# openjamoses/TOSEM-2021-Replication

Measured on NVIDIA H100. Metric: source MB/s scanned (tokenise + line-hash + classify + aggregate), higher is better.
Workload: dtype u8

## Files before the change

### tosem-2021-replication_b200/csrc/tsm_api.cu

```cuda
#include <algorithm>
#include <cstdio>
#include <cstdlib>
#include <cstring>
#include <chrono>
#include <new>
#include <utility>
#include <vector>

#include "tsm_device.cuh"

#include "tsm_scan_kernels.cuh"
#include "tsm_scan_walk.cuh"
#include "tsm_reduce_kernels.cuh"
#include "tsm_diff_kernels.cuh"
#include "tsm_blame_kernels.cuh"
#include "tsm_stmt_kernels.cuh"
#include "tsm_lines_kernels.cuh"
#include "tsm_similar_kernels.cuh"
#include "tsm_clone_kernels.cuh"
#include "tsm_case_kernels.cuh"
#include "tsm_edit_kernels.cuh"

using namespace tsm;

// ... 351 lines not shown
  rc = upload_index(c, k, st);
  if (rc != TSM_OK) return rc;
  if (c->n_files) CU(cudaMemcpyAsync(c->d_arena, k->arena, (size_t)c->arena_bytes, cudaMemcpyHostToDevice, st));
  c->resident = true;
  c->scanned = false;
  return TSM_OK;
}

static int ensure_event_buffers(tsm_ctx* c, uint32_t flags) {
  if ((flags & TSM_SCAN_ASSERT_EVENTS) && !c->d_aev)
    CU(cudaMalloc((void**)&c->d_aev, sizeof(tsm_assert_event) * (size_t)c->max_events));
  if ((flags & TSM_SCAN_HEADER_EVENTS) && !c->d_hev)
    CU(cudaMalloc((void**)&c->d_hev, sizeof(tsm_header_event) * (size_t)c->max_events));
  return TSM_OK;
}

static ScanParams make_params(const tsm_ctx* c, uint32_t flags) {
  ScanParams p{};
  p.arena = c->d_arena; p.off = c->d_off; p.len = c->d_len; p.ext = c->d_ext; p.grp = c->d_grp;
  p.n_files = c->n_files; p.n_groups = c->n_groups;
  p.unit_file = c->d_unit_file; p.unit_begin = c->d_unit_begin; p.unit_cap = c->unit_cap;
  p.ctrl = c->d_ctrl; p.stats = c->d_stats;
  p.cand = c->d_cand; p.cand_cap = (uint32_t)c->max_events;
  p.hev = c->d_hev; p.hev_cap = (uint32_t)c->max_events;
  p.aev = c->d_aev; p.aev_cap = (uint32_t)c->max_events;
  p.counts = c->d_counts; p.flags = flags; p.four = 4; p.cls_last = 1;
  return p;
}

static void launch_k_scan(const tsm_ctx* c, const ScanParams& p, bool rev_b, cudaStream_t st) {
  if (rev_b) k_scan_t<true><<<c->sms * SCAN2_CTAS_PER_SM, SCAN2_WARPS * 32, SCAN2_SMEM_B, st>>>(p);
  else k_scan_t<false><<<c->sms * SCAN2_CTAS_PER_SM, SCAN2_WARPS * 32, SCAN2_SMEM, st>>>(p);
}

struct ClassifyShape { size_t smem; uint32_t wave; };
static ClassifyShape classify_shape(tsm_ctx* c, int32_t n_groups) {
  const size_t smem = CLS_SMEM_BASE + sizeof(uint32_t) * (n_groups <= 16 ? (size_t)n_groups * TSM_K : 0);
  if (c->cls_smem != smem) {
    int per_sm = 0;
    if (cudaOccupancyMaxActiveBlocksPerMultiprocessor(&per_sm, k_classify_t<false>, 256, smem) != cudaSuccess || per_sm < 1) per_sm = 4;
    c->cls_per_sm = per_sm;
    c->cls_smem = smem;
  }
  return {smem, (uint32_t)(c->sms * c->cls_per_sm)};
}

static void launch_k_classify(const ScanParams& p, bool rev_b, uint32_t grid, size_t smem, cudaStream_t st) {
  if (rev_b) k_classify_t<true><<<grid, 256, smem, st>>>(p);
  else k_classify_t<false><<<grid, 256, smem, st>>>(p);
}

static int launch_scan(tsm_ctx* c, uint32_t flags, cudaStream_t st, const tsm_corpus* host, bool check_files_here = false) {
  int rc = ensure_event_buffers(c, flags);
  if (rc != TSM_OK) return rc;
  ScanParams p = make_params(c, flags);
  const int n = c->n_files;
  c->launches = 0;
  CU(cudaMemsetAsync(c->d_zero, 0, (size_t)(reinterpret_cast<uint8_t*>(c->d_counts) - c->d_zero) +
                     sizeof(unsigned long long) * ((size_t)(c->n_groups + 1) * TSM_K + 4), st));
  if (n) {
    std::vector<int32_t> cut{0};
    if (host) {
      int64_t slab_bytes = 32ll << 20;
      while (c->arena_bytes / slab_bytes + 1 > tsm_ctx::kMaxSlabs) slab_bytes *= 2;
      int64_t next = slab_bytes;
      for (int32_t i = 1; i < n; ++i)
        if ((int64_t)host->off[i] >= next) { cut.push_back(i); next = (int64_t)host->off[i] + slab_bytes; }
      CU(cudaEventRecord(c->ready_ev, st));
      CU(cudaStreamWaitEvent(c->copy_stream, c->ready_ev, 0));
    }
    cut.push_back(n);
    if ((int)cut.size() - 1 > tsm_ctx::kMaxSlabs) return TSM_E_LAYOUT;
    const int es = c->ev_next;
    c->ev_next = (es + 1) % tsm_ctx::kRing;
    fold_events(c, es);
    cudaEvent_t* ev = c->ev[es];
    CU(cudaEventRecord(ev[0], st));
    const int n_slabs = (int)cut.size() - 1;
    const bool rev_b = flags & TSM_SCAN_REV_B;
    const ClassifyShape cls = classify_shape(c, c->n_groups);
    for (int s = 0; s < n_slabs; ++s) {
      const int32_t f0 = cut[(size_t)s], f1 = cut[(size_t)s + 1];
      if (host) {
        if (check_files_here && s == 0) {
          const int rc0 = check_files(host, f0, f1, true, true);
          if (rc0 != TSM_OK) return rc0;
        }
        const size_t b0 = (size_t)host->off[f0], b1 = (size_t)host->off[f1];
        CU(cudaMemcpyAsync(c->d_arena + b0, host->arena + b0, b1 - b0, cudaMemcpyHostToDevice, c->copy_stream));
        CU(cudaEventRecord(c->slab_ev[s], c->copy_stream));
        CU(cudaStreamWaitEvent(st, c->slab_ev[s], 0));
        if (check_files_here && s + 1 < n_slabs) {
          const int rc1 = check_files(host, f1, cut[(size_t)s + 2], true, true);
          if (rc1 != TSM_OK) { cudaStreamSynchronize(c->copy_stream); cudaStreamSynchronize(st); return rc1; }
        }
      }
      p.slab = c->d_slab + s; p.f_begin = f0; p.f_end = f1;
      p.unit_base = (uint32_t)((host ? (int64_t)host->off[f0] : 0) / CH + f0);
      k_plan<<<(f1 - f0 + 255) / 256, 256, 0, st>>>(p);
      CU(cudaGetLastError());
      if (s == 0 && n_slabs == 1) CU(cudaEventRecord(ev[1], st));
      launch_k_scan(c, p, rev_b, st);
      CU(cudaGetLastError());
      if (s + 1 < n_slabs) {
        p.cls_last = 0;
        launch_k_classify(p, rev_b, cls.wave, cls.smem, st);
        CU(cudaGetLastError());
        p.cls_last = 1;
      }
    }
    if (n_slabs > 1) CU(cudaEventRecord(ev[1], st));
    CU(cudaEventRecord(ev[2], st));
    launch_k_classify(p, rev_b, cls.wave, cls.smem, st);
    CU(cudaGetLastError());
    CU(cudaEventRecord(ev[3], st));
    CU(cudaEventRecord(ev[4], st));
    c->ev_used[es] = (n_slabs == 1);
    c->ev_last = es;
    c->launches = 3 * n_slabs;
    CU(cudaGetLastError());
  }
  c->last_flags = flags;
  c->scanned = true;
  return TSM_OK;
}

extern "C" int tsm_scan_resident(tsm_ctx* c, uint32_t flags, void* stream) {
  if (!c) return TSM_E_ARG;
  flags &= TSM_SCAN_ASSERT_EVENTS | TSM_SCAN_HEADER_EVENTS | TSM_SCAN_REV_B;
  if (!c->resident) return TSM_E_STATE;
  CallScope call(c, (cudaStream_t)stream);
  CU(call.status);
  return launch_scan(c, flags, (cudaStream_t)stream, nullptr);
}

extern "C" int tsm_device_counts(tsm_ctx* c, void** dptr, int64_t* n_int64) {
  if (!c || !dptr || !n_int64) return TSM_E_ARG;
  if (!c->scanned) return TSM_E_STATE;
  *dptr = c->d_counts;
  *n_int64 = (int64_t)(c->n_groups + 1) * TSM_K + 4;
  return TSM_OK;
}

extern "C" int tsm_last_launch_count(tsm_ctx* c) { return c ? c->launches : 0; }

#if TSM_PHASE_CLOCKS
extern "C" int tsm_phase_clocks(unsigned long long* out, int n, int reset) {
  if (!out || n < (int)PH_N) return TSM_E_ARG;
  CU(cudaDeviceSynchronize());
  CU(cudaMemcpyFromSymbol(out, g_scan_phase_clk, sizeof(unsigned long long) * PH_N));
  if (reset) {
    const unsigned long long zero[PH_N] = {};
    CU(cudaMemcpyToSymbol(g_scan_phase_clk, zero, sizeof(zero)));
  }
  return TSM_OK;
}
#endif

extern "C" int tsm_last_kernel_ms(tsm_ctx* c, float* ms4) {
  if (!c || !ms4) return TSM_E_ARG;
  if (!c->scanned || c->n_files == 0 || c->ev_last < 0) return TSM_E_STATE;
  CU(cudaSetDevice(c->device));
  cudaEvent_t* ev = c->ev[c->ev_last];
  CU(cudaEventSynchronize(ev[4]));
  for (int i = 0; i < 4; ++i) CU(cudaEventElapsedTime(&ms4[i], ev[i], ev[i + 1]));
  return TSM_OK;
}

extern "C" int tsm_kernel_ms_stats(tsm_ctx* c, double* sum_ms4, int64_t* n_scans, int reset) {
  if (!c) return TSM_E_ARG;
  CU(cudaSetDevice(c->device));
  for (int i = 0; i < tsm_ctx::kRing; ++i) fold_events(c, i);
  if (sum_ms4) for (int k = 0; k < 4; ++k) sum_ms4[k] = c->ms_sum[k];
  if (n_scans) *n_scans = c->ms_n;
  if (reset) { for (double& v : c->ms_sum) v = 0; c->ms_n = 0; }
  return TSM_OK;
}

static int grow_event_buffers(tsm_ctx* c, int64_t need) {
  if (need <= c->max_events) return TSM_OK;
  if (need > 0xFFFFFFF0ll) return TSM_E_CAPACITY;
  unsigned long long* cand = nullptr;
  tsm_assert_event* aev = nullptr;
  tsm_header_event* hev = nullptr;
  const bool ok = cudaMalloc((void**)&cand, sizeof(unsigned long long) * (size_t)need) == cudaSuccess &&
                  (!c->d_aev || cudaMalloc((void**)&aev, sizeof(tsm_assert_event) * (size_t)need) == cudaSuccess) &&
                  (!c->d_hev || cudaMalloc((void**)&hev, sizeof(tsm_header_event) * (size_t)need) == cudaSuccess);
  if (!ok) {
    cudaGetLastError();
    cudaFree(cand); cudaFree(aev); cudaFree(hev);
    return TSM_E_CUDA;
  }
  cudaFree(c->d_cand); cudaFree(c->d_aev); cudaFree(c->d_hev);
  c->d_cand = cand; c->d_aev = aev; c->d_hev = hev;
  c->max_events = need;
  return TSM_OK;
}

static int download_tables(tsm_ctx* c, tsm_result* r, cudaStream_t st) {
  const int n = c->n_files, G = c->n_groups;
  unsigned long long* h_tot = reinterpret_cast<unsigned long long*>(c->h_ctrl + 1);
  CU(cudaMemcpyAsync(c->h_ctrl, c->d_ctrl, sizeof(Ctrl), cudaMemcpyDeviceToHost, st));
  CU(cudaMemcpyAsync(h_tot, c->d_counts + (size_t)(G + 1) * TSM_K, 4 * sizeof(unsigned long long), cudaMemcpyDeviceToHost, st));
  if (r->stats && n) CU(cudaMemcpyAsync(r->stats, c->d_stats, sizeof(tsm_file_stat) * (size_t)n, cudaMemcpyDeviceToHost, st));
  if (r->group_counts) CU(cudaMemcpyAsync(r->group_counts, c->d_counts, sizeof(int64_t) * (size_t)G * TSM_K, cudaMemcpyDeviceToHost, st));
  if (r->global_counts) CU(cudaMemcpyAsync(r->global_counts, c->d_counts + (size_t)G * TSM_K, sizeof(int64_t) * TSM_K, cudaMemcpyDeviceToHost, st));
  CU(cudaStreamSynchronize(st));
  for (int i = 0; i < 4; ++i) r->totals[i] = (int64_t)h_tot[i];
  return TSM_OK;
}

template <typename Event> static void sort_events_by_file(Event* ev, uint32_t m, int32_t n_files) {
  if (m < 2) return;
  std::vector<uint32_t> pos((size_t)n_files + 1, 0);
  for (uint32_t i = 0; i < m; ++i) pos[(size_t)ev[i].file + 1]++;
  for (int32_t f = 0; f < n_files; ++f) pos[(size_t)f + 1] += pos[(size_t)f];
  std::vector<Event> tmp(m);
  std::vector<uint32_t> at(pos.begin(), pos.end() - 1);
  for (uint32_t i = 0; i < m; ++i) tmp[at[ev[i].file]++] = ev[i];
  for (int32_t f = 0; f < n_files; ++f)
    if (pos[(size_t)f + 1] - pos[(size_t)f] > 1)
      std::sort(tmp.begin() + pos[(size_t)f], tmp.begin() + pos[(size_t)f + 1],
                [](const Event& a, const Event& b) { return a.line_off < b.line_off; });
  std::copy(tmp.begin(), tmp.end(), ev);
}

static int download(tsm_ctx* c, tsm_result* r, cudaStream_t st) {
  r->n_aev = 0; r->n_hev = 0;
  int rc = download_tables(c, r, st);
  if (rc != TSM_OK) return rc;
  if (c->h_ctrl->overflow) {
    const Ctrl& k = *c->h_ctrl;
    rc = grow_event_buffers(c, std::max<int64_t>(k.n_cand, std::max(k.n_hev, k.n_aev)));
    if (rc == TSM_OK) rc = launch_scan(c, c->last_flags, st, nullptr);
    if (rc == TSM_OK) rc = download_tables(c, r, st);
    if (rc != TSM_OK) return rc;
    if (c->h_ctrl->overflow) return TSM_E_CAPACITY;
  }
  const bool want_aev = (c->last_flags & TSM_SCAN_ASSERT_EVENTS) && r->aev, want_hev = (c->last_flags & TSM_SCAN_HEADER_EVENTS) && r->hev;
  if ((want_aev && (int64_t)c->h_ctrl->n_aev > r->aev_cap) || (want_hev && (int64_t)c->h_ctrl->n_hev > r->hev_cap)) {
    r->n_aev = c->h_ctrl->n_aev; r->n_hev = c->h_ctrl->n_hev;
    return TSM_E_CAPACITY;
  }
  if (want_aev) {
    const uint32_t m = c->h_ctrl->n_aev;
    CU(cudaMemcpyAsync(r->aev, c->d_aev, sizeof(tsm_assert_event) * (size_t)m, cudaMemcpyDeviceToHost, st));
    CU(cudaStreamSynchronize(st));
    sort_events_by_file(r->aev, m, c->n_files);
    r->n_aev = m;
  } else if (c->last_flags & TSM_SCAN_ASSERT_EVENTS) r->n_aev = c->h_ctrl->n_aev;
  if (want_hev) {
    const uint32_t m = c->h_ctrl->n_hev;
    CU(cudaMemcpyAsync(r->hev, c->d_hev, sizeof(tsm_header_event) * (size_t)m, cudaMemcpyDeviceToHost, st));
    CU(cudaStreamSynchronize(st));
    sort_events_by_file(r->hev, m, c->n_files);
    r->n_hev = m;
  } else if (c->last_flags & TSM_SCAN_HEADER_EVENTS) r->n_hev = c->h_ctrl->n_hev;
  return TSM_OK;
}

extern "C" int tsm_download(tsm_ctx* c, tsm_result* r, void* stream) {
  if (!c || !r) return TSM_E_ARG;
  if (!c->scanned) return TSM_E_STATE;
  CallScope call(c, (cudaStream_t)stream);
  CU(call.status);
  return download(c, r, (cudaStream_t)stream);
}

extern "C" int tsm_scan(tsm_ctx* c, const tsm_corpus* k, tsm_result* r, uint32_t flags, void* stream) {
  if (!c || !r) return TSM_E_ARG;
  int rc = check_corpus_head(c, k);
  if (rc != TSM_OK) return rc;
  flags &= TSM_SCAN_ASSERT_EVENTS | TSM_SCAN_HEADER_EVENTS | TSM_SCAN_REV_B;
  cudaStream_t st = (cudaStream_t)stream;
  CallScope call(c, st);
  CU(call.status);
  rc = upload_index(c, k, st);
  if (rc != TSM_OK) return rc;
  c->resident = true;
  rc = launch_scan(c, flags, st, k, true);
  if (rc != TSM_OK) { c->resident = false; c->scanned = false; return rc; }
  return download(c, r, st);
}

extern "C" int tsm_reduce(tsm_ctx* c, const uint8_t* flags, const int32_t* repo, const int32_t* case_id,
                          int32_t n_rows, int32_t n_flags, int32_t n_repos, int32_t n_cases,
                          int64_t* out, int64_t* cases_per_repo, void* stream) {
  if (!c || n_rows < 0 || n_flags < 0 || n_repos <= 0 || n_cases <= 0 || !out || (n_rows && (!flags || !repo || !case_id)))
    return TSM_E_ARG;
  for (int32_t i = 0; i < n_rows; ++i)
    if (repo[i] < 0 || repo[i] >= n_repos || case_id[i] < 0 || case_id[i] >= n_cases) return TSM_E_ARG;
  cudaStream_t st = (cudaStream_t)stream;
  CallScope call(c, st);
  CU(call.status);
  const size_t words = ((size_t)n_cases + 31) / 32;
  const size_t nbits = (size_t)(n_flags + 1) * n_repos * words;
  DevBuf b_flags, b_repo, b_case, b_bits, b_out;
  SyncGuard guard(st);
  if (!b_flags.alloc((size_t)n_rows * n_flags) || !b_repo.alloc(sizeof(int32_t) * (size_t)n_rows) ||
      !b_case.alloc(sizeof(int32_t) * (size_t)n_rows) || !b_bits.alloc(sizeof(uint32_t) * nbits) ||
      !b_out.alloc(sizeof(unsigned long long) * (size_t)(n_flags + 1) * n_repos))
    return TSM_E_CUDA;
  uint8_t* d_flags = b_flags.as<uint8_t>(); int32_t *d_repo = b_repo.as<int32_t>(), *d_case = b_case.as<int32_t>();
  uint32_t* d_bits = b_bits.as<uint32_t>();
  unsigned long long* d_out = b_out.as<unsigned long long>();
  int rc = TSM_OK;
// ... 1193 lines not shown
```

### tosem-2021-replication_b200/csrc/tsm_scan_kernels.cuh

```cuda
#pragma once
#include "tsm_device.cuh"

namespace tsm {

__constant__ uint32_t c_lut[256];
__constant__ uint32_t c_lut_b[256];
__constant__ uint32_t c_elut[256];
__device__ uint8_t c_cat_slot[TSM_CAT_SLOTS];
__device__ uint16_t c_cat_off[TSM_CAT_NAMED + 1];
__device__ char c_cat_blob[TSM_CAT_BLOB_LEN + 1];

__global__ void k_plan(ScanParams p) {
  const int f = p.f_begin + blockIdx.x * blockDim.x + threadIdx.x;
  const int lane = threadIdx.x & 31;
  if (blockIdx.x == 0 && threadIdx.x == 0) p.ctrl->cls_done = p.ctrl->n_cand;
  uint32_t nu = 0;
  if (f < p.f_end) {
    nu = ((uint32_t)p.len[f] + CH - 1) / CH;
    if (nu != 1) p.stats[f] = tsm_file_stat{0, 0, 0, 0, 0};
  }
  uint32_t incl = nu;
#pragma unroll
  for (int d = 1; d < 32; d <<= 1) {
    uint32_t t = __shfl_up_sync(0xffffffffu, incl, d);
    if (lane >= d) incl += t;
  }
  const uint32_t total = __shfl_sync(0xffffffffu, incl, 31);
  uint32_t base = 0;
  if (lane == 31 && total) base = atomicAdd(&p.slab->n_units, total);
  base = __shfl_sync(0xffffffffu, base, 31);
  uint32_t at = p.unit_base + base + incl - nu;
  for (uint32_t u = 0; u < nu; ++u, ++at) {
    if (at < p.unit_cap) { p.unit_file[at] = (uint32_t)f; p.unit_begin[at] = u * CH; }
    else p.ctrl->overflow = 1;
  }
}

__device__ __forceinline__ uint32_t nl_word(uint32_t w) {
  const uint32_t y = w ^ 0x0A0A0A0Au;
  const uint32_t t = (y & 0x7F7F7F7Fu) + 0x7F7F7F7Fu;
  const uint32_t z = ~(t | y | 0x7F7F7F7Fu);
  return (z * 0x00204081u) >> 28;
}
__device__ __forceinline__ uint32_t spaces_of(unsigned long long w) {
  const unsigned long long x = w ^ 0x2020202020202020ull, k7 = 0x7F7F7F7F7F7F7F7Full;
  const unsigned long long nz = (((x & k7) + k7) | x) & ~k7;
  return nz ? ((uint32_t)__ffsll((long long)nz) - 1u) >> 3 : 8u;
}
struct SmemByte {
  const uint8_t* b;
  __device__ __forceinline__ uint32_t operator()(uint32_t i) const { return b[i]; }
  __device__ __forceinline__ unsigned long long load8(uint32_t i) const {
    const uint32_t a = i & ~7u, sh = 8u * (i & 7u);
    const unsigned long long lo = *reinterpret_cast<const unsigned long long*>(b + a);
    const unsigned long long hi = *reinterpret_cast<const unsigned long long*>(b + a + 8);
    return sh ? (lo >> sh) | (hi << (64u - sh)) : lo;
  }
  __device__ __forceinline__ uint32_t spaces8(uint32_t i) const { return spaces_of(load8(i)); }
};
struct HbmByte {
  const uint8_t* b;
  __device__ __forceinline__ uint32_t operator()(uint32_t i) const { return __ldg(b + i); }
  __device__ __forceinline__ unsigned long long load8(uint32_t i) const {
    const unsigned long long* w = reinterpret_cast<const unsigned long long*>(b) + (i >> 3);
    const uint32_t sh = 8u * (i & 7u);
    const unsigned long long lo = __ldg(w), hi = __ldg(w + 1);
    return sh ? (lo >> sh) | (hi << (64u - sh)) : lo;
  }
  __device__ __forceinline__ uint32_t spaces8(uint32_t i) const { return spaces_of(load8(i)); }
};
struct Accum { uint32_t lines, asserts, hdrs, fixes; unsigned long long digest; };

__device__ __forceinline__ uint32_t warp_reserve(uint32_t* counter, uint32_t n, int lane) {
  uint32_t base = 0;
  if (lane == 0 && n) base = atomicAdd(counter, n);
  return __shfl_sync(0xffffffffu, base, 0);
}

__device__ __forceinline__ const uint32_t* scan_lut() {
  extern __shared__ __align__(128) uint8_t smem[];
  return reinterpret_cast<const uint32_t*>(smem);
}

__device__ __forceinline__ void issue_load(const ScanParams& p, uint8_t* buf, uint64_t* bar, uint32_t fo,
                                           uint32_t size, uint32_t cb) {
  const uint32_t lb = cb ? cb - PRE : 0u;
  const uint32_t le = min(cb + CH + EXT, size);
  const uint32_t bytes = (le - lb + 15u) & ~15u;
  mbar_expect_tx(bar, bytes);
  bulk_load(buf + PRE - (cb - lb), p.arena + (size_t)fo + lb, bytes, bar);
}

struct Unit { uint32_t u, f, cb, fo, size; int ext; };

__device__ __forceinline__ Unit claim_unit(const ScanParams& p, uint32_t n_units, int lane) {
  Unit x{0, 0, 0, 0, 0, 0};
  if (lane == 0) x.u = atomicAdd(&p.slab->work, 1u);
  x.u = __shfl_sync(0xffffffffu, x.u, 0);
  if (x.u < n_units) {
    x.f = p.unit_file[p.unit_base + x.u];
    x.cb = p.unit_begin[p.unit_base + x.u];
    x.fo = (uint32_t)p.off[x.f];
    x.size = (uint32_t)p.len[x.f];
    x.ext = p.ext[x.f];
  }
  return x;
}

constexpr uint32_t CC_W = 1, CC_IDENT = 2, CC_STOP = 4;
constexpr uint32_t CLS_CAT_OFF_N = (TSM_CAT_NAMED + 2) & ~1u;
constexpr uint32_t CLS_CAT_WORDS = ((TSM_CAT_SLOTS + 2 * CLS_CAT_OFF_N + TSM_CAT_BLOB_LEN + 15) / 16) * 4;
constexpr uint32_t CLS_SMEM_BASE = 4 * (512 + CLS_CAT_WORDS + 4 * 1024 + 4);
constexpr uint32_t E_FIRST = (1u << 0) | (1u << 5) | (1u << 9) | (1u << 17) | (1u << 21) | (1u << 23) | (1u << 25) |
                             (1u << 27) | (1u << 29) | (1u << 30);

struct FileBytes {
  const unsigned long long* base; uint32_t cur_blk; unsigned long long w;
  uint32_t blk0; unsigned long long w0, w1, w2, w3;
  __device__ __forceinline__ FileBytes(const uint8_t* b, uint32_t first_byte)
      : base(reinterpret_cast<const unsigned long long*>(b)), cur_blk(0xFFFFFFFFu), w(0), blk0(first_byte >> 3) {
    w0 = __ldg(base + blk0); w1 = __ldg(base + blk0 + 1); w2 = __ldg(base + blk0 + 2); w3 = __ldg(base + blk0 + 3);
  }
  __device__ __forceinline__ unsigned long long word(uint32_t blk) const {
    const uint32_t d = blk - blk0;
    if (d < 4u) return d < 2u ? (d == 0u ? w0 : w1) : (d == 2u ? w2 : w3);
    return __ldg(base + blk);
  }
  __device__ __forceinline__ uint32_t get(uint32_t i) {
    const uint32_t blk = i >> 3;
    if (blk != cur_blk) { w = word(blk); cur_blk = blk; }
    return (uint32_t)(w >> (8u * (i & 7u))) & 0xFFu;
  }
  __device__ __forceinline__ unsigned long long get8(uint32_t i) const {
    const uint32_t blk = i >> 3, sh = 8u * (i & 7u);
    const unsigned long long lo = word(blk);
    if (sh == 0) return lo;
    return (lo >> sh) | (word(blk + 1) << (64u - sh));
  }
};

__device__ __forceinline__ unsigned long long low_bytes(unsigned long long v, uint32_t n) {
  return n >= 8 ? v : (v & ((1ull << (8u * n)) - 1ull));
}

__device__ __forceinline__ int stem_lookup(FileBytes& rd, uint32_t s, uint32_t n) {
  if (n < 2 || n > 9) return 0;
  const unsigned long long v = low_bytes(rd.get8(s), n);
  const uint32_t c9 = n == 9 ? rd.get(s + 8) : 0u;
  switch (n) {
    case 2:
      if (v == 0x5145ull) return 1;
      if (v == 0x454Eull) return 2;
      if (v == 0x5447ull) return 5;
      if (v == 0x4547ull) return 6;
      if (v == 0x544Cull) return 7;
      if (v == 0x454Cull) return 8;
      return 0;
    case 4:
      if (v == 0x45555254ull) return 3;
      if (v == 0x5241454Eull) return 9;
      return 0;
    case 5:
      if (v == 0x45534C4146ull) return 4;
      if (v == 0x574F524854ull) return 12;
      return 0;
    case 8: return v == 0x51455F54414F4C46ull ? 10 : 0;
    case 9: return (v == 0x455F454C42554F44ull && c9 == 'Q') ? 11 : 0;
    default: return 0;
  }
}

__device__ __forceinline__ int bare_assert_category(FileBytes& rd, uint32_t e0, uint32_t en, const uint32_t* elut, int deflt = 3,
                                                    bool not_prefix = true) {
  if (not_prefix && en >= 4 && (uint32_t)rd.get8(e0) == 0x20746F6Eu) return 2;
  uint32_t D = 0, A = 0;
  for (uint32_t a = 0; a < en; a += 8) {
    unsigned long long w = rd.get8(e0 + a);
    if (en - a < 8) w &= (1ull << (8u * (en - a))) - 1ull;
    const uint32_t lo = (uint32_t)w, hi = (uint32_t)(w >> 32);
#pragma unroll
    for (int k = 0; k < 4; ++k) { D = ((D + D) | E_FIRST) & elut[__byte_perm(lo, 0, 0x4440 + k)]; A |= D; }
#pragma unroll
    for (int k = 0; k < 4; ++k) { D = ((D + D) | E_FIRST) & elut[__byte_perm(hi, 0, 0x4440 + k)]; A |= D; }
  }
  if (((A & (1u << 4)) && (A & (1u << 8))) || (A & (1u << 16))) return 4;
  if (A & (1u << 20)) return 3;
  if (A & (1u << 22)) return 1;
  if (A & (1u << 24)) return 2;
  if (A & (1u << 26)) return 8;
  if (A & (1u << 28)) return 6;
  if (A & (1u << 29)) return 7;
  if (A & (1u << 30)) return 5;
  return deflt;
}

__device__ __noinline__ bool ident_eq(FileBytes& rd, uint32_t s, uint32_t n, const char* name, uint32_t len) {
  if (n != len) return false;
  for (uint32_t k = 0; k < len; ++k)
    if (rd.get(s + k) != (uint8_t)name[k]) return false;
  return true;
}

constexpr uint32_t BQ_CAP = 1024;

#ifndef TSM_CLS_MINB
#define TSM_CLS_MINB 1
#endif
template <bool REVB>
__global__ void __launch_bounds__(256, TSM_CLS_MINB) k_classify_t(ScanParams p) {
  extern __shared__ __align__(16) uint32_t csm[];
  uint32_t* cls = csm;
  uint32_t* elut = csm + 256;
  uint8_t* cat_slot = reinterpret_cast<uint8_t*>(csm + 512);
  uint16_t* cat_off = reinterpret_cast<uint16_t*>(cat_slot + TSM_CAT_SLOTS);
  uint8_t* cat_blob = reinterpret_cast<uint8_t*>(cat_off + CLS_CAT_OFF_N);
  uint4* bq = reinterpret_cast<uint4*>(csm + 512 + CLS_CAT_WORDS);
  uint32_t* bqn = csm + 512 + CLS_CAT_WORDS + 4 * BQ_CAP;
  uint32_t* hist = bqn + 4;
  const bool use_smem = p.n_groups <= 16;
  for (int i = threadIdx.x; i < 256; i += blockDim.x) {
    const uint32_t c = (uint32_t)i;
    cls[i] = (is_w(c) ? CC_W : 0u) | (is_ident(c) ? CC_IDENT : 0u) | ((c == '(' || c == '\n') ? CC_STOP : 0u);
    elut[i] = c_elut[i];
  }
  for (int i = threadIdx.x; i < TSM_CAT_SLOTS; i += blockDim.x) cat_slot[i] = c_cat_slot[i];
  for (int i = threadIdx.x; i < TSM_CAT_NAMED + 1; i += blockDim.x) cat_off[i] = c_cat_off[i];
  for (int i = threadIdx.x; i < TSM_CAT_BLOB_LEN; i += blockDim.x) cat_blob[i] = (uint8_t)c_cat_blob[i];
  if (use_smem) for (int i = threadIdx.x; i < p.n_groups * TSM_K; i += blockDim.x) hist[i] = 0;
  if (threadIdx.x == 0) *bqn = 0;
  __syncthreads();
  auto count = [&](uint32_t f, int cat) {
    const uint32_t g = p.grp ? p.grp[f] : 0u;
    if (use_smem) atomicAdd(&hist[g * TSM_K + cat], 1u);
    else {
      atomicAdd(&p.counts[(size_t)g * TSM_K + cat], 1ull);
      atomicAdd(&p.counts[(size_t)p.n_groups * TSM_K + cat], 1ull);
    }
  };
  const uint32_t n = min(p.ctrl->n_cand, p.cand_cap), n0 = min(p.ctrl->cls_done, n);
  const bool want_ev = (p.flags & TSM_SCAN_ASSERT_EVENTS) != 0;
  constexpr bool revb = REVB;
  for (uint32_t i = n0 + blockIdx.x * blockDim.x + threadIdx.x; i < n; i += gridDim.x * blockDim.x) {
    const unsigned long long cd = p.cand[i];
    const uint32_t f = (uint32_t)(cd >> 32), line_off = (uint32_t)cd;
    const uint32_t size = (uint32_t)p.len[f];
    FileBytes rd(p.arena + (size_t)(uint32_t)p.off[f], line_off);
    uint32_t q = line_off;
    while (q < size && (cls[rd.get(q)] & CC_W)) ++q;
    const uint32_t t0 = q;
    uint32_t stop = size;
    for (uint32_t wb = t0 & ~7u; wb < size; wb += 8) {
      unsigned long long w = rd.word(wb >> 3);
      const unsigned long long x1 = w ^ 0x2828282828282828ull, x2 = w ^ 0x0A0A0A0A0A0A0A0Aull;
      const unsigned long long k7 = 0x7F7F7F7F7F7F7F7Full;
      unsigned long long z = (~(((x1 & k7) + k7) | x1 | k7)) | (~(((x2 & k7) + k7) | x2 | k7));
      if (wb < t0) z &= ~0ull << (8u * (t0 - wb));
      if (z) { stop = wb + ((uint32_t)__ffsll((long long)z) - 1u) / 8u; break; }
    }
    stop = min(stop, size);
    uint32_t last = stop;
    while (last > t0 && (cls[rd.get(last - 1)] & CC_W)) --last;
    uint32_t Ls = last;
    while (Ls > t0 && (cls[rd.get(Ls - 1)] & CC_IDENT)) --Ls;
    uint32_t tlen = last - t0;
    const uint32_t tlen_a = tlen, Ln = last - Ls;
    int cat = 0;
    bool done = false;
    uint32_t def_e0 = 0, def_en = 0;
    if (revb) {
      const bool macro = ident_eq(rd, Ls, Ln, "BOOST_CHECK", 11) || ident_eq(rd, Ls, Ln, "NTA_CHECK", 9);
      const bool bare6 = tlen == 6 && low_bytes(rd.get8(t0), 6) == 0x747265737361ull;
      const bool full = macro || p.ext[f] == TSM_EXT_JAVA;
      uint32_t fe = last;
      if (full || ((macro || bare6) && stop < size && rd.get(stop) == '(')) {
        uint32_t le = stop;
        while (le < size && rd.get(le) != '\n') ++le;
        fe = le;
        while (fe > t0 && (cls[rd.get(fe - 1)] & CC_W)) --fe;
      }
      if (ident_eq(rd, Ls, Ln, "BOOST_CHECK_EQUAL", 17)) { cat = 1; done = true; }
      else if ((macro || bare6) && stop < size && rd.get(stop) == '(') {
        uint32_t x = stop + 1;
        while (x < fe && (cls[rd.get(x)] & CC_W)) ++x;
        if (x < fe && rd.get(x) == '!' && !(x + 1 < fe && rd.get(x + 1) == '=')) cat = 4;
        else cat = bare_assert_category(rd, x, fe > x ? fe - x : 0u, elut, macro ? 0 : 3, false);
        done = true;
      }
      if (full) tlen = fe - t0;
    }
    if (Ln >= 7) {
      const unsigned long long h7 = low_bytes(rd.get8(Ls), 7);
      if (h7 == 0x5F544345505845ull || h7 == 0x5F545245535341ull) { cat = stem_lookup(rd, Ls + 7, Ln - 7); done = true; }
    }
    if (!done && tlen_a >= 6) {
      const unsigned long long h = rd.get8(t0);
      const bool a6 = low_bytes(h, 6) == 0x747265737361ull;
      if (a6 && tlen_a == 6) { cat = 3; done = true; }
      else if (a6 && tlen_a >= 8 && ((h >> 48) & 0xFF) == 0x20) {
        done = true;
        def_e0 = t0 + 7; def_en = tlen_a - 7;
      }
    }
    if (!done && Ln >= 6) {
      const unsigned long long h = rd.get8(Ls);
      if (low_bytes(h, 6) == 0x747265737361ull) {
        if (Ln == 7 && ((h >> 48) & 0xFF) == '_') cat = 3;
        else {
          cat = TSM_CAT_OTHER;
          uint32_t hh = 0x811C9DC5u;
          for (uint32_t j = 0; j < Ln; j += 8) {
            unsigned long long w = rd.get8(Ls + j);
            const uint32_t nb = min(8u, Ln - j);
#pragma unroll
            for (uint32_t k = 0; k < 8; ++k) {
              if (k < nb) hh = (hh ^ ((uint32_t)w & 0xFFu)) * 0x01000193u;
              w >>= 8;
            }
          }
          const int id = cat_slot[(hh * TSM_CAT_HASH_MULT) >> 23];
          if (id && (uint32_t)(cat_off[id + 1] - cat_off[id]) == Ln) {
            const uint8_t* name = cat_blob + cat_off[id];
            bool ok = true;
            for (uint32_t j = 0; j < Ln; j += 8) {
              unsigned long long w = rd.get8(Ls + j);
              const uint32_t nb = min(8u, Ln - j);
              for (uint32_t k = 0; k < nb; ++k) { ok &= ((uint32_t)w & 0xFFu) == (uint32_t)name[j + k]; w >>= 8; }
            }
            if (ok) cat = id;
          }
        }
      }
    }
    uint32_t ev_slot = 0xFFFFFFFFu;
    if (want_ev) {
      unsigned long long hacc = 0; uint32_t hr = 0;
      for (uint32_t j = 0; j < tlen; ++j) {
        hacc = fold61(hacc + rotl61((unsigned long long)rd.get(t0 + j), hr));
        hr += 8; if (hr >= 61) hr -= 61;
      }
      const uint32_t slot = atomicAdd(&p.ctrl->n_aev, 1u);
      if (slot < p.aev_cap) {
        tsm_assert_event ev;
        ev.file = f; ev.line_off = line_off; ev.stmt_off = t0;
        ev.stmt_len = (uint16_t)min(tlen, 65535u); ev.cat = (uint16_t)cat;
        ev.ident_off = Ls; ev.ident_len = (uint16_t)min(Ln, 65535u); ev.pad = 0;
        ev.stmt_hash = mix_hash(canon61(hacc), tlen);
        p.aev[slot] = ev;
        ev_slot = slot;
      } else p.ctrl->overflow = 1;
    }
    if (def_en) {
      const uint32_t slot = atomicAdd(bqn, 1u);
      if (slot < BQ_CAP) { bq[slot] = make_uint4(f, def_e0, def_en, ev_slot); continue; }
      cat = bare_assert_category(rd, def_e0, def_en, elut);
      if (ev_slot != 0xFFFFFFFFu) p.aev[ev_slot].cat = (uint16_t)cat;
    }
    count(f, cat);
  }
  __syncthreads();
  {
    const uint32_t nq = min(*bqn, BQ_CAP);
    for (uint32_t t = threadIdx.x; t < nq; t += blockDim.x) {
      const uint4 e = bq[t];
      FileBytes rd(p.arena + (size_t)(uint32_t)p.off[e.x], e.y);
      const int cat = bare_assert_category(rd, e.y, e.z, elut);
      if (e.w != 0xFFFFFFFFu) p.aev[e.w].cat = (uint16_t)cat;
      count(e.x, cat);
    }
  }
  if (p.cls_last) {
    unsigned long long t0 = 0, t1 = 0, t2 = 0, t3 = 0;
    for (int f = blockIdx.x * blockDim.x + threadIdx.x; f < p.n_files; f += gridDim.x * blockDim.x) {
      const tsm_file_stat s = p.stats[f];
      t0 += s.n_lines; t1 += s.n_assert; t2 += s.n_headers; t3 += s.n_fixture;
    }
#pragma unroll
    for (int d = 16; d; d >>= 1) {
      t0 += __shfl_xor_sync(0xffffffffu, t0, d); t1 += __shfl_xor_sync(0xffffffffu, t1, d);
      t2 += __shfl_xor_sync(0xffffffffu, t2, d); t3 += __shfl_xor_sync(0xffffffffu, t3, d);
    }
    if ((threadIdx.x & 31) == 0) {
      unsigned long long* tot = p.counts + (size_t)(p.n_groups + 1) * TSM_K;
      if (t0) atomicAdd(&tot[0], t0);
      if (t1) atomicAdd(&tot[1], t1);
      if (t2) atomicAdd(&tot[2], t2);
      if (t3) atomicAdd(&tot[3], t3);
    }
  }
  if (use_smem) {
    __syncthreads();
    for (int i = threadIdx.x; i < p.n_groups * TSM_K; i += blockDim.x) {
      const uint32_t v = hist[i];
      if (v) {
        atomicAdd(&p.counts[i], (unsigned long long)v);
        atomicAdd(&p.counts[(size_t)p.n_groups * TSM_K + (i & (TSM_K - 1))], (unsigned long long)v);
      }
    }
  }
}

template __global__ void k_classify_t<false>(ScanParams);
template __global__ void k_classify_t<true>(ScanParams);

}
```

Before: 617,400.

## Replace per-byte class-table scans with SWAR word-wide blank/ident run search

The classify kernel's per-byte whitespace and identifier scans, which looked up a shared-memory class table, are replaced with SWAR 64-bit masks and ctz/clz run searches over 8-byte words. The shared class table is removed, which shrinks the shared-memory layout. Shared-memory setup copies of the category slot table and blob are vectorised, and the name-compare loop is unrolled. Optional compile-gated clock instrumentation is also added, and it compiles to no-ops by default.

```diff
diff --git a/tosem-2021-replication_b200/csrc/tsm_api.cu b/tosem-2021-replication_b200/csrc/tsm_api.cu
--- a/tosem-2021-replication_b200/csrc/tsm_api.cu
+++ b/tosem-2021-replication_b200/csrc/tsm_api.cu
@@ -527,6 +527,19 @@
   if (reset) {
     const unsigned long long zero[PH_N] = {};
     CU(cudaMemcpyToSymbol(g_scan_phase_clk, zero, sizeof(zero)));
+  }
+  return TSM_OK;
+}
+#endif
+
+#if TSM_CLS_CLOCKS
+extern "C" int tsm_cls_clocks(unsigned long long* out, int n, int reset) {
+  if (!out || n < (int)CLS_CLK_N) return TSM_E_ARG;
+  CU(cudaDeviceSynchronize());
+  CU(cudaMemcpyFromSymbol(out, g_cls_clk, sizeof(unsigned long long) * CLS_CLK_N));
+  if (reset) {
+    const unsigned long long zero[CLS_CLK_N] = {};
+    CU(cudaMemcpyToSymbol(g_cls_clk, zero, sizeof(zero)));
   }
   return TSM_OK;
 }
diff --git a/tosem-2021-replication_b200/csrc/tsm_scan_kernels.cuh b/tosem-2021-replication_b200/csrc/tsm_scan_kernels.cuh
--- a/tosem-2021-replication_b200/csrc/tsm_scan_kernels.cuh
+++ b/tosem-2021-replication_b200/csrc/tsm_scan_kernels.cuh
@@ -6,9 +6,9 @@
 __constant__ uint32_t c_lut[256];
 __constant__ uint32_t c_lut_b[256];
 __constant__ uint32_t c_elut[256];
-__device__ uint8_t c_cat_slot[TSM_CAT_SLOTS];
+__device__ __align__(16) uint8_t c_cat_slot[TSM_CAT_SLOTS];
 __device__ uint16_t c_cat_off[TSM_CAT_NAMED + 1];
-__device__ char c_cat_blob[TSM_CAT_BLOB_LEN + 1];
+__device__ __align__(4) char c_cat_blob[TSM_CAT_BLOB_LEN + 1];
 
 __global__ void k_plan(ScanParams p) {
   const int f = p.f_begin + blockIdx.x * blockDim.x + threadIdx.x;
@@ -107,10 +107,9 @@
   return x;
 }
 
-constexpr uint32_t CC_W = 1, CC_IDENT = 2, CC_STOP = 4;
 constexpr uint32_t CLS_CAT_OFF_N = (TSM_CAT_NAMED + 2) & ~1u;
 constexpr uint32_t CLS_CAT_WORDS = ((TSM_CAT_SLOTS + 2 * CLS_CAT_OFF_N + TSM_CAT_BLOB_LEN + 15) / 16) * 4;
-constexpr uint32_t CLS_SMEM_BASE = 4 * (512 + CLS_CAT_WORDS + 4 * 1024 + 4);
+constexpr uint32_t CLS_SMEM_BASE = 4 * (256 + CLS_CAT_WORDS + 4 * 1024 + 4);
 constexpr uint32_t E_FIRST = (1u << 0) | (1u << 5) | (1u << 9) | (1u << 17) | (1u << 21) | (1u << 23) | (1u << 25) |
                              (1u << 27) | (1u << 29) | (1u << 30);
 
@@ -141,6 +140,58 @@
 
 __device__ __forceinline__ unsigned long long low_bytes(unsigned long long v, uint32_t n) {
   return n >= 8 ? v : (v & ((1ull << (8u * n)) - 1ull));
+}
+
+constexpr unsigned long long SW_H = 0x8080808080808080ull, SW_L7 = 0x7F7F7F7F7F7F7F7Full, SW_1 = 0x0101010101010101ull;
+__host__ __device__ __forceinline__ unsigned long long sw_eq(unsigned long long y, uint32_t c) {
+  return ~((y ^ (SW_1 * c)) + SW_L7) & SW_H;
+}
+__host__ __device__ __forceinline__ unsigned long long sw_in(unsigned long long y, uint32_t lo, uint32_t hi) {
+  return (y + SW_1 * (0x80u - lo)) & ~(y + SW_1 * (0x7Fu - hi)) & SW_H;
+}
+__host__ __device__ __forceinline__ unsigned long long blank_mask(unsigned long long w) {
+  const unsigned long long y = w & SW_L7;
+  return (sw_eq(y, 0x20) | (sw_in(y, 0x09, 0x0D) & ~sw_eq(y, 0x0A))) & ~w;
+}
+__host__ __device__ __forceinline__ unsigned long long ident_mask(unsigned long long w) {
+  const unsigned long long y = w & SW_L7;
+  return (sw_in(y | (SW_1 * 0x20u), 'a', 'z') | sw_in(y, '0', '9') | sw_eq(y, '_')) & ~w;
+}
+__host__ __device__ __forceinline__ uint32_t sw_ctz(unsigned long long x) {
+#ifdef __CUDA_ARCH__
+  return (uint32_t)__ffsll((long long)x) - 1u;
+#else
+  return (uint32_t)__builtin_ctzll(x);
+#endif
+}
+__host__ __device__ __forceinline__ uint32_t sw_clz(unsigned long long x) {
+#ifdef __CUDA_ARCH__
+  return (uint32_t)__clzll((long long)x);
+#else
+  return (uint32_t)__builtin_clzll(x);
+#endif
+}
+template <class Word, class Mask>
+__host__ __device__ __forceinline__ uint32_t run_fwd(const Word& word, uint32_t b, uint32_t hi, Mask mask) {
+  if (b >= hi) return b;
+  while (b < hi) {
+    const uint32_t j = b & 7u;
+    const unsigned long long out = (~mask(word(b >> 3)) & SW_H) >> (8u * j);
+    if (out) { b += sw_ctz(out) >> 3; break; }
+    b += 8u - j;
+  }
+  return b < hi ? b : hi;
+}
+template <class Word, class Mask>
+__host__ __device__ __forceinline__ uint32_t run_back(const Word& word, uint32_t e, uint32_t lo, Mask mask) {
+  if (e <= lo) return e;
+  while (e > lo) {
+    const uint32_t j = (e - 1u) & 7u;
+    const unsigned long long out = (~mask(word((e - 1u) >> 3)) & SW_H) << (8u * (7u - j));
+    if (out) { e -= sw_clz(out) >> 3; break; }
+    e -= j + 1u;
+  }
+  return e > lo ? e : lo;
 }
 
 __device__ __forceinline__ int stem_lookup(FileBytes& rd, uint32_t s, uint32_t n) {
@@ -203,32 +254,72 @@
 
 constexpr uint32_t BQ_CAP = 1024;
 
+#ifndef TSM_CLS_CLOCKS
+#define TSM_CLS_CLOCKS 0
+#endif
+enum ClsPhase { CP_PROLOGUE, CP_FETCH, CP_BOUNDS, CP_RULES, CP_COUNT, CP_BARRIER, CP_DEFERRED, CP_TOTALS, CP_FLUSH, CP_N };
+enum ClsLoop { CL_CAND, CL_INDENT, CL_STOP, CL_STRIP, CL_IDENT, CL_RULE_WORDS, CL_DEFERRED, CL_DEFERRED_WORDS, CL_N };
+constexpr uint32_t CLS_CLK_N = CP_N + 2 * CL_N;
+#if TSM_CLS_CLOCKS
+__device__ unsigned long long g_cls_clk[CLS_CLK_N];
+#endif
+struct ClsClock {
+#if TSM_CLS_CLOCKS
+  uint32_t* tab;
+  long long t;
+  __device__ __forceinline__ void mark(int ph, uint32_t dep = 0u) {
+    if (dep == 0x9E3779B9u) tab[CLS_CLK_N] = dep;
+    const uint32_t m = __activemask();
+    __syncwarp(m);
+    const long long now = clock64();
+    if ((threadIdx.x & 31) == (uint32_t)__ffs(m) - 1u) atomicAdd(tab + ph, (uint32_t)(now - t));
+    t = now;
+  }
+  __device__ __forceinline__ void trips(int loop, uint32_t n) {
+    const uint32_t m = __activemask();
+    const uint32_t s = __reduce_add_sync(m, n), x = __reduce_max_sync(m, n);
+    if ((threadIdx.x & 31) == (uint32_t)__ffs(m) - 1u && x) {
+      atomicAdd(tab + CP_N + loop, s);
+      atomicAdd(tab + CP_N + CL_N + loop, x);
+    }
+  }
+#else
+  __device__ __forceinline__ void mark(int, uint32_t = 0u) {}
+  __device__ __forceinline__ void trips(int, uint32_t) {}
+#endif
+};
+
 #ifndef TSM_CLS_MINB
 #define TSM_CLS_MINB 1
 #endif
 template <bool REVB>
 __global__ void __launch_bounds__(256, TSM_CLS_MINB) k_classify_t(ScanParams p) {
   extern __shared__ __align__(16) uint32_t csm[];
-  uint32_t* cls = csm;
-  uint32_t* elut = csm + 256;
-  uint8_t* cat_slot = reinterpret_cast<uint8_t*>(csm + 512);
+  uint32_t* elut = csm;
+  uint8_t* cat_slot = reinterpret_cast<uint8_t*>(csm + 256);
   uint16_t* cat_off = reinterpret_cast<uint16_t*>(cat_slot + TSM_CAT_SLOTS);
   uint8_t* cat_blob = reinterpret_cast<uint8_t*>(cat_off + CLS_CAT_OFF_N);
-  uint4* bq = reinterpret_cast<uint4*>(csm + 512 + CLS_CAT_WORDS);
-  uint32_t* bqn = csm + 512 + CLS_CAT_WORDS + 4 * BQ_CAP;
+  uint4* bq = reinterpret_cast<uint4*>(csm + 256 + CLS_CAT_WORDS);
+  uint32_t* bqn = csm + 256 + CLS_CAT_WORDS + 4 * BQ_CAP;
   uint32_t* hist = bqn + 4;
   const bool use_smem = p.n_groups <= 16;
-  for (int i = threadIdx.x; i < 256; i += blockDim.x) {
-    const uint32_t c = (uint32_t)i;
-    cls[i] = (is_w(c) ? CC_W : 0u) | (is_ident(c) ? CC_IDENT : 0u) | ((c == '(' || c == '\n') ? CC_STOP : 0u);
-    elut[i] = c_elut[i];
-  }
-  for (int i = threadIdx.x; i < TSM_CAT_SLOTS; i += blockDim.x) cat_slot[i] = c_cat_slot[i];
+  ClsClock ck;
+#if TSM_CLS_CLOCKS
+  __shared__ uint32_t cls_clk_tab[CLS_CLK_N + 1];
+  ck.tab = cls_clk_tab;
+  ck.t = clock64();
+  for (int i = threadIdx.x; i < (int)CLS_CLK_N; i += blockDim.x) cls_clk_tab[i] = 0u;
+#endif
+  for (int i = threadIdx.x; i < 256; i += blockDim.x) elut[i] = c_elut[i];
+  for (int i = threadIdx.x; i < TSM_CAT_SLOTS / 16; i += blockDim.x)
+    reinterpret_cast<uint4*>(cat_slot)[i] = reinterpret_cast<const uint4*>(c_cat_slot)[i];
   for (int i = threadIdx.x; i < TSM_CAT_NAMED + 1; i += blockDim.x) cat_off[i] = c_cat_off[i];
-  for (int i = threadIdx.x; i < TSM_CAT_BLOB_LEN; i += blockDim.x) cat_blob[i] = (uint8_t)c_cat_blob[i];
+  for (int i = threadIdx.x; i < (TSM_CAT_BLOB_LEN + 1) / 4; i += blockDim.x)
+    reinterpret_cast<uint32_t*>(cat_blob)[i] = reinterpret_cast<const uint32_t*>(c_cat_blob)[i];
   if (use_smem) for (int i = threadIdx.x; i < p.n_groups * TSM_K; i += blockDim.x) hist[i] = 0;
   if (threadIdx.x == 0) *bqn = 0;
   __syncthreads();
+  ck.mark(CP_PROLOGUE);
   auto count = [&](uint32_t f, int cat) {
     const uint32_t g = p.grp ? p.grp[f] : 0u;
     if (use_smem) atomicAdd(&hist[g * TSM_K + cat], 1u);
@@ -240,14 +331,16 @@
   const uint32_t n = min(p.ctrl->n_cand, p.cand_cap), n0 = min(p.ctrl->cls_done, n);
   const bool want_ev = (p.flags & TSM_SCAN_ASSERT_EVENTS) != 0;
   constexpr bool revb = REVB;
+  uint32_t n_iter = 0;
   for (uint32_t i = n0 + blockIdx.x * blockDim.x + threadIdx.x; i < n; i += gridDim.x * blockDim.x) {
+    ++n_iter;
     const unsigned long long cd = p.cand[i];
     const uint32_t f = (uint32_t)(cd >> 32), line_off = (uint32_t)cd;
     const uint32_t size = (uint32_t)p.len[f];
     FileBytes rd(p.arena + (size_t)(uint32_t)p.off[f], line_off);
-    uint32_t q = line_off;
-    while (q < size && (cls[rd.get(q)] & CC_W)) ++q;
-    const uint32_t t0 = q;
+    ck.mark(CP_FETCH, (uint32_t)(rd.w0 ^ rd.w1 ^ rd.w2 ^ rd.w3) ^ size);
+    auto word = [&rd](uint32_t blk) { return rd.word(blk); };
+    const uint32_t t0 = run_fwd(word, line_off, size, blank_mask);
     uint32_t stop = size;
     for (uint32_t wb = t0 & ~7u; wb < size; wb += 8) {
       unsigned long long w = rd.word(wb >> 3);
@@ -258,12 +351,16 @@
       if (z) { stop = wb + ((uint32_t)__ffsll((long long)z) - 1u) / 8u; break; }
     }
     stop = min(stop, size);
-    uint32_t last = stop;
-    while (last > t0 && (cls[rd.get(last - 1)] & CC_W)) --last;
-    uint32_t Ls = last;
-    while (Ls > t0 && (cls[rd.get(Ls - 1)] & CC_IDENT)) --Ls;
+    const uint32_t last = run_back(word, stop, t0, blank_mask);
+    const uint32_t Ls = run_back(word, last, t0, ident_mask);
     uint32_t tlen = last - t0;
     const uint32_t tlen_a = tlen, Ln = last - Ls;
+    ck.trips(CL_INDENT, (t0 - (line_off & ~7u)) / 8u + 1u);
+    ck.trips(CL_STOP, (stop - (t0 & ~7u)) / 8u + 1u);
+    ck.trips(CL_STRIP, (stop + 7u) / 8u - last / 8u);
+    ck.trips(CL_IDENT, (last + 7u) / 8u - Ls / 8u);
+    ck.mark(CP_BOUNDS);
+    uint32_t rule_words = 0;
     int cat = 0;
     bool done = false;
     uint32_t def_e0 = 0, def_en = 0;
@@ -275,13 +372,11 @@
       if (full || ((macro || bare6) && stop < size && rd.get(stop) == '(')) {
         uint32_t le = stop;
         while (le < size && rd.get(le) != '\n') ++le;
-        fe = le;
-        while (fe > t0 && (cls[rd.get(fe - 1)] & CC_W)) --fe;
+        fe = run_back(word, le, t0, blank_mask);
       }
       if (ident_eq(rd, Ls, Ln, "BOOST_CHECK_EQUAL", 17)) { cat = 1; done = true; }
       else if ((macro || bare6) && stop < size && rd.get(stop) == '(') {
-        uint32_t x = stop + 1;
-        while (x < fe && (cls[rd.get(x)] & CC_W)) ++x;
+        const uint32_t x = run_fwd(word, stop + 1, fe, blank_mask);
         if (x < fe && rd.get(x) == '!' && !(x + 1 < fe && rd.get(x + 1) == '=')) cat = 4;
         else cat = bare_assert_category(rd, x, fe > x ? fe - x : 0u, elut, macro ? 0 : 3, false);
         done = true;
@@ -308,6 +403,7 @@
         else {
           cat = TSM_CAT_OTHER;
           uint32_t hh = 0x811C9DC5u;
+          rule_words += (Ln + 7u) / 8u;
           for (uint32_t j = 0; j < Ln; j += 8) {
             unsigned long long w = rd.get8(Ls + j);
             const uint32_t nb = min(8u, Ln - j);
@@ -321,16 +417,23 @@
           if (id && (uint32_t)(cat_off[id + 1] - cat_off[id]) == Ln) {
             const uint8_t* name = cat_blob + cat_off[id];
             bool ok = true;
+            rule_words += (Ln + 7u) / 8u;
             for (uint32_t j = 0; j < Ln; j += 8) {
               unsigned long long w = rd.get8(Ls + j);
               const uint32_t nb = min(8u, Ln - j);
-              for (uint32_t k = 0; k < nb; ++k) { ok &= ((uint32_t)w & 0xFFu) == (uint32_t)name[j + k]; w >>= 8; }
+#pragma unroll
+              for (uint32_t k = 0; k < 8; ++k) {
+                if (k < nb) ok &= ((uint32_t)w & 0xFFu) == (uint32_t)name[j + k];
+                w >>= 8;
+              }
             }
             if (ok) cat = id;
           }
         }
       }
     }
+    ck.trips(CL_RULE_WORDS, rule_words);
+    ck.mark(CP_RULES);
     uint32_t ev_slot = 0xFFFFFFFFu;
     if (want_ev) {
       unsigned long long hacc = 0; uint32_t hr = 0;
@@ -349,24 +452,35 @@
         ev_slot = slot;
       } else p.ctrl->overflow = 1;
     }
+    bool queued = false;
     if (def_en) {
       const uint32_t slot = atomicAdd(bqn, 1u);
-      if (slot < BQ_CAP) { bq[slot] = make_uint4(f, def_e0, def_en, ev_slot); continue; }
-      cat = bare_assert_category(rd, def_e0, def_en, elut);
-      if (ev_slot != 0xFFFFFFFFu) p.aev[ev_slot].cat = (uint16_t)cat;
-    }
-    count(f, cat);
-  }
+      if (slot < BQ_CAP) { bq[slot] = make_uint4(f, def_e0, def_en, ev_slot); queued = true; }
+      else {
+        cat = bare_assert_category(rd, def_e0, def_en, elut);
+        if (ev_slot != 0xFFFFFFFFu) p.aev[ev_slot].cat = (uint16_t)cat;
+      }
+    }
+    if (!queued) count(f, cat);
+    ck.mark(CP_COUNT);
+  }
+  ck.trips(CL_CAND, n_iter);
   __syncthreads();
+  ck.mark(CP_BARRIER);
   {
     const uint32_t nq = min(*bqn, BQ_CAP);
+    uint32_t nd = 0, dw = 0;
     for (uint32_t t = threadIdx.x; t < nq; t += blockDim.x) {
       const uint4 e = bq[t];
+      ++nd; dw += (e.z + 7u) / 8u;
       FileBytes rd(p.arena + (size_t)(uint32_t)p.off[e.x], e.y);
       const int cat = bare_assert_category(rd, e.y, e.z, elut);
       if (e.w != 0xFFFFFFFFu) p.aev[e.w].cat = (uint16_t)cat;
       count(e.x, cat);
     }
+    ck.trips(CL_DEFERRED, nd);
+    ck.trips(CL_DEFERRED_WORDS, dw);
+    ck.mark(CP_DEFERRED);
   }
   if (p.cls_last) {
     unsigned long long t0 = 0, t1 = 0, t2 = 0, t3 = 0;
@@ -387,6 +501,7 @@
       if (t3) atomicAdd(&tot[3], t3);
     }
   }
+  ck.mark(CP_TOTALS);
   if (use_smem) {
     __syncthreads();
     for (int i = threadIdx.x; i < p.n_groups * TSM_K; i += blockDim.x) {
@@ -397,6 +512,11 @@
       }
     }
   }
+  ck.mark(CP_FLUSH);
+#if TSM_CLS_CLOCKS
+  __syncthreads();
+  for (int i = threadIdx.x; i < (int)CLS_CLK_N; i += blockDim.x) atomicAdd(&g_cls_clk[i], (unsigned long long)cls_clk_tab[i]);
+#endif
 }
 
 template __global__ void k_classify_t<false>(ScanParams);
```

Result: faster. 627,500, median of 6 (+1.6%).
